# WeGoToMars/indexed_bzip2

Hardware: AMD Instinct MI355X
Metric: decompressed MB/s (whole node), 2 GiB Silesia bz2-9 (higher is better)
Workload: dtype u8

## Files before the change

indexed_bzip2_amd/csrc/bz2_hscan.hip.h:

```cpp
#pragma once

#include "bz2_stage1.hip.h"

namespace bz2gpu
{
constexpr uint32_t SCAN_LUT_BITS = 10;
constexpr uint32_t SCAN_LUT_SIZE = 1u << SCAN_LUT_BITS;
constexpr uint32_t SCAN_MAX_SPAN = 1024;
constexpr uint32_t SCAN_ROWS = SCAN_MAX_SPAN / 64;
constexpr uint32_t GROUP_SYMS = 50;
constexpr uint32_t MAX_SCAN_GROUPS = 18002;
constexpr uint32_t LEN_STOP = 0x80u;
constexpr uint32_t SYM_THREADS = 128;
constexpr uint32_t SYM_CHUNKS = 4;

struct alignas( 16 ) HuffTables
{
    uint16_t lut[6][SCAN_LUT_SIZE];
    uint16_t perm[6][264];
    uint32_t first[6][24];
    uint32_t count[6][24];
    uint32_t offs[6][24];
    uint32_t minmax[8];
};
static_assert( sizeof( HuffTables ) % 16 == 0 );

struct ScanMeta
{
    uint64_t pos_base;
    uint32_t size_bits;
    uint32_t n_groups;
    uint32_t terminal;
    uint32_t symbol_count;
    uint32_t pad[2];
};

constexpr uint32_t SCAN_RING_ENTRIES = 256;
constexpr uint32_t SCAN_RING_MIRROR = 40;

constexpr uint32_t LEV_ENTRIES = SCAN_MAX_SPAN + 16;
constexpr uint32_t LEV_BYTES = 2 * LEV_ENTRIES;

struct alignas( 16 ) ScanSlot
{
    uint16_t lev[3 * LEV_ENTRIES];

    __device__ __forceinline__ uint8_t* bytes() { return reinterpret_cast<uint8_t*>( lev ); }
    __device__ __forceinline__ uint16_t& at( uint32_t array, uint32_t entry ) { return lev[array * LEV_ENTRIES + entry]; }
};

struct ScanHeader
{
    uint64_t enc_size, pos_base;
    int32_t  status, is_eos, is_eof;
    uint32_t active, header_crc, orig_ptr, symbol_count, n_sel, size_bits, p0, n_words;
};

template<uint32_t K>
struct ScanShared
{
    uint8_t  lenlut[6][SCAN_LUT_SIZE];
    uint32_t limit[6][24];
    uint32_t eob_lo[6], eob_hi[6];
    uint32_t minmax[6];
    uint32_t ring[2 * ( SCAN_RING_ENTRIES + SCAN_RING_MIRROR )];
    ScanHeader hdr;
    union alignas( 16 ) {
        struct {
            uint16_t lut[SCAN_LUT_SIZE];
            uint32_t first[24], count[24], offs[24], running[24];
            uint16_t perm[264];
            uint16_t bitmap[16];
            uint8_t  lens[264];
            uint8_t  sym_to_byte[256];
        } build;
        ScanSlot slot[K > 1 ? 2 : 1];
    };
};

template<uint32_t RING = SCAN_RING_ENTRIES>
__device__ __forceinline__ void
ring_put( uint32_t* ring, uint32_t index, uint32_t raw )
{
    const uint32_t value = be32( raw );
    const uint32_t e1 = index & ( RING - 1 );
    const uint32_t e0 = ( index - 1 ) & ( RING - 1 );
    ring[2 * e1 + 1] = value;
    ring[2 * e0] = value;
    if ( e1 < SCAN_RING_MIRROR ) ring[2 * ( RING + e1 ) + 1] = value;
    if ( e0 < SCAN_RING_MIRROR ) ring[2 * ( RING + e0 )] = value;
}

template<uint32_t K>
__device__ __forceinline__ void
scan_sync()
{
    if ( K > 1 ) __syncthreads(); else wave_sync();
// ... 928 lines not shown
        const uint32_t fullGroups = terminal ? nGroups - 1 : nGroups;
        BlockMeta mt;
        mt.enc_off = start;
        mt.enc_size = sh.hdr.enc_size;
        mt.decoded_size = 0;
        mt.out_off = 0;
        mt.header_crc = sh.hdr.header_crc;
        mt.computed_crc = 0xFFFFFFFFu;
        mt.n = 0;
        mt.orig_ptr = sh.hdr.orig_ptr;
        mt.nsym = fullGroups * GROUP_SYMS;
        mt.is_eos = sh.hdr.is_eos;
        mt.is_eof = sh.hdr.is_eof;
        mt.status = status;
        mt.seg_stride = MIN_SEG_STRIDE;
        mt.nseg = 0;
        mt.walk_ok = 0;
        mt.cycle_len = 0;
        mt.nchain = 0;
        mt.pad = 0;
        meta[b] = mt;
        HuffMeta hm;
        hm.n_stored = fullGroups * GROUP_SYMS;
        hm.symbol_count = sh.hdr.symbol_count;
        hm.status = status;
        hm.active = active;
        hmeta[b] = hm;
        ScanMeta sm;
        sm.pos_base = posBase;
        sm.size_bits = sizeBits;
        sm.n_groups = nGroups;
        sm.terminal = terminal;
        sm.symbol_count = sh.hdr.symbol_count;
        smeta[b] = sm;
    }
}


template<uint32_t THREADS>
struct alignas( 16 ) SymShared
{
    HuffTables tabs;
    uint16_t stage[THREADS * GROUP_SYMS];
};

template<uint32_t THREADS = SYM_THREADS>
__global__ __launch_bounds__( THREADS ) void
k_hsym( const uint32_t* __restrict__   in_words,
        BlockMeta* __restrict__        meta,
        HuffMeta* __restrict__         hmeta,
        const ScanMeta* __restrict__   smeta,
        const uint8_t* __restrict__    sel_buf,
        const HuffTables* __restrict__ tab_buf,
        const uint32_t* __restrict__   gpos_buf,
        uint16_t* __restrict__         sym_buf )
{
    extern __shared__ __attribute__( ( aligned( 16 ) ) ) uint8_t ldsAtLaunch[];
    SymShared<THREADS>& sh = *reinterpret_cast<SymShared<THREADS>*>( ldsAtLaunch );
    const uint32_t b = blockIdx.y;
    const ScanMeta sm = smeta[b];
    if ( blockIdx.x * THREADS * SYM_CHUNKS >= sm.n_groups ) return;
    const uint32_t tid = threadIdx.x;
    {
        const uint4* const src = reinterpret_cast<const uint4*>( tab_buf + b );
        uint4* const dst = reinterpret_cast<uint4*>( &sh.tabs );
        for ( uint32_t k = tid; k < sizeof( HuffTables ) / 16; k += THREADS ) dst[k] = src[k];
    }
    __syncthreads();

    for ( uint32_t chunk = 0; chunk < SYM_CHUNKS; ++chunk ) {
    const uint32_t g0 = ( blockIdx.x * SYM_CHUNKS + chunk ) * THREADS;
    if ( g0 >= sm.n_groups ) return;
    const uint32_t gi = g0 + tid;
    const uint32_t eob = sm.symbol_count + 1;
    if ( gi < sm.n_groups ) {
        const uint32_t t = sel_buf[(size_t)b * SEL_STRIDE + gi];
        const uint32_t* const words = in_words + ( sm.pos_base >> 5 );
        uint32_t pos = gpos_buf[(size_t)b * GPOS_STRIDE + gi];
        const bool last = sm.terminal && gi + 1 == sm.n_groups;
        uint32_t w = pos >> 5;
        uint64_t buf = ( ( (uint64_t)be32( words[w] ) << 32 ) | be32( words[w + 1] ) ) << ( pos & 31u );
        uint32_t have = 64 - ( pos & 31u );
        w += 2;
        const uint16_t* const lut = sh.tabs.lut[t];
        const uint32_t mm = sh.tabs.minmax[t];
        const uint32_t maxLen = mm >> 8;
        uint16_t* const out = sh.stage + tid * GROUP_SYMS;
        uint32_t cnt = 0;
        int32_t status = ST_OK;
        bool finished = false;
        for ( uint32_t j = 0; j < GROUP_SYMS; ++j ) {
            if ( have <= 32 ) {
                buf |= (uint64_t)be32( words[w] ) << ( 32 - have );
                have += 32;
                ++w;
            }
            uint32_t e = lut[(uint32_t)( buf >> ( 64 - SCAN_LUT_BITS ) )];
            uint32_t len = e & 31u, sym = e >> 5;
            if ( len == 0 ) {
                const uint32_t v20 = (uint32_t)( buf >> 44 );
                for ( uint32_t l = SCAN_LUT_BITS + 1; l <= maxLen; ++l ) {
                    const uint32_t d = ( v20 >> ( 20 - l ) ) - sh.tabs.first[t][l];
                    if ( d < sh.tabs.count[t][l] ) {
                        len = l;
                        sym = sh.tabs.perm[t][sh.tabs.offs[t][l] + d];
                        break;
                    }
                }
            }
            if ( last ) {
                if ( len == 0 ) {
                    status = pos + maxLen > sm.size_bits ? ST_EOF : ST_INVALID_CODE;
                    break;
                }
                if ( pos + len > sm.size_bits ) {
                    status = ST_EOF;
                    break;
                }
            }
            pos += len;
            buf <<= len;
            have -= len;
            if ( last && sym == eob ) {
                finished = true;
                break;
            }
            out[j] = (uint16_t)sym;
            ++cnt;
        }
        if ( last ) {
            const uint32_t stored = gi * GROUP_SYMS + cnt;
            if ( !finished && status == ST_OK ) status = ST_INVALID_CODE;
            hmeta[b].n_stored = stored;
            hmeta[b].status = status;
            meta[b].nsym = stored + ( finished ? 1u : 0u );
            meta[b].status = status;
            meta[b].enc_size = sm.pos_base + pos - meta[b].enc_off;
        }
    }
    __syncthreads();
    {
        const uint32_t nHere = sm.n_groups - g0 < THREADS ? sm.n_groups - g0 : THREADS;
        const uint32_t units = ( nHere * GROUP_SYMS * 2 + 15 ) / 16;
        uint4* const dst = reinterpret_cast<uint4*>( sym_buf + (size_t)b * SYM_STRIDE + (size_t)g0 * GROUP_SYMS );
        const uint4* const src = reinterpret_cast<const uint4*>( sh.stage );
        for ( uint32_t k = tid; k < units; k += THREADS ) dst[k] = src[k];
    }
    __syncthreads();
    }
}
}
```

indexed_bzip2_amd/csrc/bz2_kernels.hip.h:

```cpp
#pragma once

#include <hip/hip_runtime.h>
#include <stdint.h>

#include "bz2_scratch.hpp"

namespace bz2gpu
{
constexpr uint32_t MAX_N = 900000;
constexpr uint32_t MIN_SEG_STRIDE = 16;
constexpr uint32_t MARK = 0x80000000u;
constexpr uint32_t LF_MASK = 0xFFFFFu;
constexpr uint32_t INVALID_OFF = 0xFFFFFFFFu;

enum Status : int32_t {
    ST_OK = 0, ST_EOF = 1, ST_BAD_MAGIC = 2, ST_RANDOMIZED = 3, ST_ORIGPTR_RANGE = 4, ST_GROUP_COUNT = 5,
    ST_SELECTOR_COUNT = 6, ST_SELECTOR_UNARY = 7, ST_CODE_LENGTH = 8, ST_HUFFMAN_LENGTHS = 9,
    ST_SELECTOR_OVERRUN = 10, ST_INVALID_CODE = 11, ST_RUN_OVERFLOW = 12, ST_DATA_OVERFLOW = 13,
    ST_ORIGPTR_DATA = 14, ST_CRC = 15
};

struct BlockMeta
{
    uint64_t enc_off;
// ... 97 lines not shown
    }

    __device__ __forceinline__ void
    skip( uint32_t k )
    {
        buf <<= k;
        n -= k;
        pos += k;
    }

    __device__ __forceinline__ uint32_t
    read( uint32_t k )
    {
        refill();
        if ( pos + k > size_bits ) {
            eof = true;
        }
        const uint32_t v = peek( k );
        skip( k );
        return v;
    }
};

__global__ __launch_bounds__( 256 ) void
k_find_magic( const uint32_t* __restrict__ words, uint64_t size_bits, uint64_t magic48,
              uint64_t* __restrict__ found, uint32_t capacity, uint32_t* __restrict__ counter )
{
    const uint64_t nStartWords = ( size_bits + 31 ) >> 5;
    const uint64_t stride = (uint64_t)gridDim.x * 256;
    for ( uint64_t w = (uint64_t)blockIdx.x * 256 + threadIdx.x; w < nStartWords; w += stride ) {
        const uint64_t hi = ( (uint64_t)be32( words[w] ) << 32 ) | be32( words[w + 1] );
        const uint64_t lo = (uint64_t)be32( words[w + 2] ) << 32;
#pragma unroll 4
        for ( uint32_t s = 0; s < 32; ++s ) {
            const uint64_t window = s == 0 ? hi : ( ( hi << s ) | ( lo >> ( 64 - s ) ) );
            if ( ( window >> 16 ) == magic48 ) {
                const uint64_t offset = w * 32 + s;
                if ( offset + 48 <= size_bits ) {
                    const uint32_t slot = atomicAdd( counter, 1u );
                    if ( slot < capacity ) found[slot] = offset;
                }
            }
        }
    }
}

__device__ __forceinline__ uint64_t
match_any( uint32_t key, int bits, bool valid )
{
    const uint64_t all = __ballot( valid );
    uint32_t lo = 0, hi = 0;
    int b = 0;
    for ( ; b + 1 < bits; b += 2 ) {
        const uint32_t minus0 = (uint32_t)__builtin_amdgcn_sbfe( (int)key, b, 1 );
        const uint32_t minus1 = (uint32_t)__builtin_amdgcn_sbfe( (int)key, b + 1, 1 );
        const uint64_t bal0 = __ballot( minus0 != 0 );
        const uint64_t bal1 = __ballot( minus1 != 0 );
        lo = lo | ( (uint32_t)bal0 ^ minus0 ) | ( (uint32_t)bal1 ^ minus1 );
        hi = hi | ( (uint32_t)( bal0 >> 32 ) ^ minus0 ) | ( (uint32_t)( bal1 >> 32 ) ^ minus1 );
    }
    if ( b < bits ) {
        const uint32_t minusBit = (uint32_t)__builtin_amdgcn_sbfe( (int)key, b, 1 );
        const uint64_t bal = __ballot( minusBit != 0 );
        lo |= (uint32_t)bal ^ minusBit;
        hi |= (uint32_t)( bal >> 32 ) ^ minusBit;
    }
    return all & ~( ( (uint64_t)hi << 32 ) | lo );
}

__device__ __forceinline__ uint64_t
match_any_runs( uint32_t key, bool valid )
{
    const uint32_t first = (uint32_t)__builtin_amdgcn_readfirstlane( (int)key );
    if ( __ballot( valid && key != first ) == 0 ) return __ballot( valid );
    return match_any( key, 8, valid );
}

__device__ __forceinline__ uint32_t
popc_below( uint64_t mask, uint32_t lane )
{
    return __popcll( mask & ( ( 1ull << lane ) - 1ull ) );
}

__global__ __launch_bounds__( 1024 ) void
k_bwt_build( const BlockMeta* __restrict__ meta,
             const uint8_t* __restrict__   l_buf,
             uint32_t* __restrict__        tab_buf )
{
    __shared__ uint32_t hist[BWT_WAVES][256];
    __shared__ uint32_t tot[256];
    const uint32_t b = blockIdx.x;
    const BlockMeta mt = meta[b];
    if ( !mt.walk_ok ) return;
    const uint32_t N = mt.n, origPtr = mt.orig_ptr, stride = mt.seg_stride;
    const uint8_t* const L = l_buf + (size_t)b * L_STRIDE;
    uint32_t* const tab = tab_buf + (size_t)b * TAB_STRIDE;
    const uint32_t tid = threadIdx.x, wave = tid >> 6, lane = tid & 63;

    uint32_t chunk = ( N + BWT_WAVES - 1 ) / BWT_WAVES;
    chunk = ( chunk + 255u ) & ~255u;
    const uint32_t begin = wave * chunk < N ? wave * chunk : N;
    const uint32_t end = begin + chunk < N ? begin + chunk : N;

    for ( uint32_t i = tid; i < BWT_WAVES * 256; i += 1024 ) ( &hist[0][0] )[i] = 0;
    __syncthreads();

    for ( uint32_t base = begin; base < end; base += 256 ) {
        const uint32_t i = base + 4 * lane;
        if ( i < end ) {
            const uint32_t v = *reinterpret_cast<const uint32_t*>( L + i );
            const uint32_t nb = end - i < 4 ? end - i : 4;
            for ( uint32_t k = 0; k < nb; ++k ) atomicAdd( &hist[wave][( v >> ( 8 * k ) ) & 0xFF], 1u );
        }
    }
    __syncthreads();
    if ( tid < 256 ) {
        uint32_t run = 0;
        for ( int w = 0; w < BWT_WAVES; ++w ) {
            const uint32_t t = hist[w][tid];
            hist[w][tid] = run;
            run += t;
        }
        tot[tid] = run;
    }
    __syncthreads();
    if ( tid < 64 ) {
        uint32_t v0 = tot[4 * tid], v1 = tot[4 * tid + 1], v2 = tot[4 * tid + 2], v3 = tot[4 * tid + 3];
        const uint32_t s = v0 + v1 + v2 + v3;
        uint32_t incl = s;
        for ( int d = 1; d < 64; d <<= 1 ) {
            const uint32_t o = __shfl_up( incl, d );
            if ( (int)tid >= d ) incl += o;
        }
        uint32_t excl = incl - s;
        tot[4 * tid] = excl; excl += v0;
        tot[4 * tid + 1] = excl; excl += v1;
        tot[4 * tid + 2] = excl; excl += v2;
        tot[4 * tid + 3] = excl;
    }
    __syncthreads();
    if ( tid < 256 ) {
        const uint32_t c = tot[tid];
        for ( int w = 0; w < BWT_WAVES; ++w ) hist[w][tid] += c;
    }
    __syncthreads();

    uint32_t rem = ( begin + lane ) % stride;
    const uint32_t remStep = 64u % stride;
    for ( uint32_t base4 = begin; base4 < end; base4 += 256 ) {
        uint32_t keys[4];
#pragma unroll
        for ( uint32_t u = 0; u < 4; ++u ) keys[u] = L[base4 + 64 * u + lane];
#pragma unroll
        for ( uint32_t u = 0; u < 4; ++u ) {
            const uint32_t i = base4 + 64 * u + lane;
            const bool valid = i < end;
            const uint32_t key = valid ? keys[u] : 0u;
            const uint64_t same = match_any_runs( key, valid );
            const uint32_t rank = popc_below( same, lane );
            uint32_t basePos = 0;
            if ( valid ) basePos = hist[wave][key];
            if ( valid ) {
                const uint32_t lf = basePos + rank;
                const bool mark = ( rem == 0 ) || ( i == origPtr );
                tab[i] = ( lf << 8 ) | key | ( mark ? MARK : 0u );
                if ( rank == 0 ) hist[wave][key] = basePos + (uint32_t)__popcll( same );
            }
            rem += remStep;
            if ( rem >= stride ) rem -= stride;
        }
    }
}

__device__ __forceinline__ void
bwt_chunk_range( uint32_t N, uint32_t slices, uint32_t slice, uint32_t wave, uint32_t& begin, uint32_t& end )
{
    uint32_t chunk = ( N + slices * BWT_WAVES - 1 ) / ( slices * BWT_WAVES );
    chunk = ( chunk + 255u ) & ~255u;
    const uint32_t index = slice * BWT_WAVES + wave;
    begin = index * chunk < N ? index * chunk : N;
    end = begin + chunk < N ? begin + chunk : N;
}

__global__ __launch_bounds__( 1024 ) void
k_bwt_count( const BlockMeta* __restrict__ meta,
             const uint8_t* __restrict__   l_buf,
             uint32_t* __restrict__        counts,
             uint32_t                      slices )
{
    __shared__ uint32_t hist[BWT_WAVES][256];
    const uint32_t b = blockIdx.y, slice = blockIdx.x;
    const BlockMeta mt = meta[b];
    if ( !mt.walk_ok ) return;
    const uint8_t* const L = l_buf + (size_t)b * L_STRIDE;
    const uint32_t tid = threadIdx.x, wave = tid >> 6, lane = tid & 63;
    uint32_t begin, end;
    bwt_chunk_range( mt.n, slices, slice, wave, begin, end );
    for ( uint32_t i = tid; i < BWT_WAVES * 256; i += 1024 ) ( &hist[0][0] )[i] = 0;
    __syncthreads();
    for ( uint32_t base = begin; base < end; base += 256 ) {
        const uint32_t i = base + 4 * lane;
        if ( i < end ) {
            const uint32_t v = *reinterpret_cast<const uint32_t*>( L + i );
            const uint32_t nb = end - i < 4 ? end - i : 4;
            for ( uint32_t k = 0; k < nb; ++k ) atomicAdd( &hist[wave][( v >> ( 8 * k ) ) & 0xFF], 1u );
        }
    }
    __syncthreads();
    uint32_t* const out = counts + (size_t)b * BWT_COUNTS_PER_BLOCK + (size_t)slice * BWT_WAVES * 256;
    for ( uint32_t i = tid; i < BWT_WAVES * 256; i += 1024 ) out[i] = ( &hist[0][0] )[i];
}

__global__ __launch_bounds__( 1024 ) void
k_bwt_rank( const BlockMeta* __restrict__ meta,
            const uint8_t* __restrict__   l_buf,
            uint32_t* __restrict__        tab_buf,
            const uint32_t* __restrict__  counts,
            uint32_t                      slices )
{
    __shared__ uint32_t hist[BWT_WAVES][256];
    __shared__ uint32_t tot[256];
    const uint32_t b = blockIdx.y, slice = blockIdx.x;
    const BlockMeta mt = meta[b];
    if ( !mt.walk_ok ) return;
    const uint32_t N = mt.n, origPtr = mt.orig_ptr, stride = mt.seg_stride;
    const uint8_t* const L = l_buf + (size_t)b * L_STRIDE;
    uint32_t* const tab = tab_buf + (size_t)b * TAB_STRIDE;
    const uint32_t tid = threadIdx.x, wave = tid >> 6, lane = tid & 63;
    if ( tid < 256 ) {
        const uint32_t* const of = counts + (size_t)b * BWT_COUNTS_PER_BLOCK + tid;
        uint32_t run = 0;
        for ( uint32_t c = 0; c < slices * BWT_WAVES; ++c ) {
            const uint32_t t = of[(size_t)c * 256];
            if ( c / BWT_WAVES == slice ) hist[c % BWT_WAVES][tid] = run;
            run += t;
        }
        tot[tid] = run;
    }
    __syncthreads();
    if ( tid < 64 ) {
        uint32_t v0 = tot[4 * tid], v1 = tot[4 * tid + 1], v2 = tot[4 * tid + 2], v3 = tot[4 * tid + 3];
        const uint32_t s4 = v0 + v1 + v2 + v3;
        uint32_t incl = s4;
        for ( int d = 1; d < 64; d <<= 1 ) {
            const uint32_t o = __shfl_up( incl, d );
            if ( (int)tid >= d ) incl += o;
        }
        uint32_t excl = incl - s4;
        tot[4 * tid] = excl; excl += v0;
        tot[4 * tid + 1] = excl; excl += v1;
        tot[4 * tid + 2] = excl; excl += v2;
        tot[4 * tid + 3] = excl;
    }
    __syncthreads();
    if ( tid < 256 ) {
        const uint32_t c = tot[tid];
        for ( int w = 0; w < BWT_WAVES; ++w ) hist[w][tid] += c;
    }
    __syncthreads();

    uint32_t begin, end;
    bwt_chunk_range( N, slices, slice, wave, begin, end );
    uint32_t rem = ( begin + lane ) % stride;
    const uint32_t remStep = 64u % stride;
    for ( uint32_t base4 = begin; base4 < end; base4 += 256 ) {
        uint32_t keys[4];
#pragma unroll
        for ( uint32_t u = 0; u < 4; ++u ) keys[u] = L[base4 + 64 * u + lane];
#pragma unroll
        for ( uint32_t u = 0; u < 4; ++u ) {
            const uint32_t i = base4 + 64 * u + lane;
            const bool valid = i < end;
            const uint32_t key = valid ? keys[u] : 0u;
            const uint64_t same = match_any_runs( key, valid );
            const uint32_t rank = popc_below( same, lane );
            uint32_t basePos = 0;
            if ( valid ) basePos = hist[wave][key];
            if ( valid ) {
                const uint32_t lf = basePos + rank;
                const bool mark = ( rem == 0 ) || ( i == origPtr );
                tab[i] = ( lf << 8 ) | key | ( mark ? MARK : 0u );
                if ( rank == 0 ) hist[wave][key] = basePos + (uint32_t)__popcll( same );
            }
            rem += remStep;
            if ( rem >= stride ) rem -= stride;
        }
    }
}

__global__ __launch_bounds__( 256 ) void
k_replicate( const BlockMeta* __restrict__ meta,
             uint8_t*                      r_buf,
             uint8_t*                      tmp_buf,
// ... 434 lines not shown
```

indexed_bzip2_amd/csrc/bz2_walk.hip.h:

```cpp
#pragma once

#include "bz2_kernels.hip.h"

namespace bz2gpu
{
constexpr uint32_t WALK_THREADS = 256;
constexpr uint32_t WALK_QUEUES = 8;
constexpr uint32_t EMIT_THREADS = 256;
constexpr uint32_t EMIT_TILES = 4;
constexpr uint32_t EMIT_STAGE = 16384;

struct WalkPlan
{
    uint32_t q_begin[WALK_QUEUES + 1];
    uint32_t q_total[WALK_QUEUES];
    uint32_t ctr[WALK_QUEUES];
    uint32_t pad[15];
};

__global__ __launch_bounds__( 256 ) void
k_walk_plan( const BlockMeta* __restrict__ meta, uint32_t n, WalkPlan* plan, uint32_t* blk, uint32_t* pre )
{
    __shared__ uint32_t begin[WALK_QUEUES + 1];
    const uint32_t t = threadIdx.x;
    if ( t == 0 ) {
        uint32_t acc = 0;
        for ( uint32_t q = 0; q < WALK_QUEUES; ++q ) {
            begin[q] = acc;
            acc += q < n ? ( n - q + WALK_QUEUES - 1 ) / WALK_QUEUES : 0;
        }
        begin[WALK_QUEUES] = acc;
    }
    __syncthreads();
    if ( t <= WALK_QUEUES ) plan->q_begin[t] = begin[t];
    if ( t < WALK_QUEUES ) {
        uint32_t idx = begin[t], acc = 0;
        for ( uint32_t i = t; i < n; i += WALK_QUEUES ) {
            blk[idx] = i;
            pre[idx] = acc;
            acc += meta[i].walk_ok ? meta[i].nseg : 0u;
            ++idx;
        }
        plan->q_total[t] = acc;
        plan->ctr[t] = 0;
    }
}

constexpr uint32_t LINK_THREADS = 256;
constexpr uint32_t LINK_SPLIT = 128;
constexpr uint32_t LINK_MAX_SUB = KMAX / LINK_SPLIT + 2;

struct alignas( 16 ) LinkShared
{
    uint16_t ssucc[SEG_STRIDE];
    uint32_t subLen[LINK_MAX_SUB];
    uint16_t subNext[LINK_MAX_SUB];
    uint32_t subOff[LINK_MAX_SUB];
    uint32_t subCnt[LINK_MAX_SUB];
    uint32_t subRank[LINK_MAX_SUB];
};

__device__ __forceinline__ void
link_block( BlockMeta*                   meta,
            const uint32_t* __restrict__ seg_len,
            const uint32_t* __restrict__ seg_succ,
            uint2* __restrict__          chain,
            uint16_t* __restrict__       ssucc,
            uint32_t* __restrict__       subLen,
            uint16_t* __restrict__       subNext,
            uint32_t* __restrict__       subOff,
            uint32_t* __restrict__       subCnt,
            uint32_t* __restrict__       subRank )
{
    const uint32_t b = blockIdx.x;
    const BlockMeta mt = meta[b];
    if ( !mt.walk_ok ) return;
    const uint32_t nseg = mt.nseg, N = mt.n, stride = mt.seg_stride, origPtr = mt.orig_ptr;
    const uint32_t k0 = ( N + stride - 1 ) / stride;
    const size_t base = (size_t)b * SEG_STRIDE;
    const uint32_t first = ( origPtr % stride != 0 ) ? k0 : origPtr / stride;
    const uint32_t tid = threadIdx.x;

    for ( uint32_t j = tid; j < nseg; j += LINK_THREADS ) {
        const uint32_t s = seg_succ[base + j];
        ssucc[j] = (uint16_t)( s < nseg ? s : 0xFFFFu );
    }
    const uint32_t nSplit = ( nseg + LINK_SPLIT - 1 ) / LINK_SPLIT;
    const bool firstExtra = first % LINK_SPLIT != 0;
    const uint32_t nSub = nSplit + ( firstExtra ? 1u : 0u );
    const auto splitterOf = [&] ( uint32_t seg ) -> uint32_t {
        if ( seg == first && firstExtra ) return nSplit;
        return seg % LINK_SPLIT == 0 ? seg / LINK_SPLIT : 0xFFFFu;
    };
    for ( uint32_t s = tid; s < LINK_MAX_SUB; s += LINK_THREADS ) subOff[s] = INVALID_OFF;
    __syncthreads();

    constexpr uint32_t AHEAD = 8;
    for ( uint32_t s = tid; s < nSub; s += LINK_THREADS ) {
        uint32_t cur = s < nSplit ? s * LINK_SPLIT : first;
        uint32_t sum = 0, steps = 0, nextSub = 0xFFFFu;
        bool more = true;
        while ( more ) {
            uint32_t nodes[AHEAD];
            uint32_t m = 0;
#pragma unroll
            for ( uint32_t k = 0; k < AHEAD; ++k ) {
                nodes[k] = cur;
                if ( more ) {
                    m = k + 1;
                    cur = ssucc[cur];
                    ++steps;
                    if ( cur == 0xFFFFu || steps > nseg ) {
                        more = false;
                    } else {
                        nextSub = splitterOf( cur );
                        more = nextSub == 0xFFFFu;
                    }
                }
            }
#pragma unroll
            for ( uint32_t k = 0; k < AHEAD; ++k ) {
                if ( k < m ) sum += seg_len[base + nodes[k]];
            }
        }
        subLen[s] = sum;
        subCnt[s] = steps;
        subNext[s] = (uint16_t)nextSub;
    }
    __syncthreads();

    if ( tid == 0 ) {
        const uint32_t start = firstExtra ? nSplit : first / LINK_SPLIT;
        uint32_t s = start, off = 0, visited = 0, rank = 0;
        bool ok = true;
        do {
            subOff[s] = off;
            subRank[s] = rank;
            off += subLen[s];
            rank += subCnt[s];
            s = subNext[s];
            ++visited;
            if ( s == 0xFFFFu || visited > nSub || off > N ) { ok = false; break; }
        } while ( s != start );
        meta[b].cycle_len = off;
        meta[b].nchain = rank;
        if ( !ok || off == 0 ) {
            meta[b].status = ST_CRC;
            meta[b].walk_ok = 0;
        }
    }
    __syncthreads();

    for ( uint32_t s = tid; s < nSub; s += LINK_THREADS ) {
        uint32_t off = subOff[s];
        if ( off == INVALID_OFF ) continue;
        uint32_t cur = s < nSplit ? s * LINK_SPLIT : first;
        uint32_t steps = 0;
        uint32_t rank = subRank[s];
        bool more = true;
        while ( more ) {
            uint32_t nodes[AHEAD], lens[AHEAD];
            uint32_t m = 0;
#pragma unroll
            for ( uint32_t k = 0; k < AHEAD; ++k ) {
                nodes[k] = cur;
                if ( more ) {
                    m = k + 1;
                    cur = ssucc[cur];
                    ++steps;
                    more = !( cur == 0xFFFFu || steps > nseg || splitterOf( cur ) != 0xFFFFu );
                }
            }
#pragma unroll
            for ( uint32_t k = 0; k < AHEAD; ++k ) lens[k] = k < m ? seg_len[base + nodes[k]] : 0u;
#pragma unroll
            for ( uint32_t k = 0; k < AHEAD; ++k ) {
                if ( k < m ) {
                    const uint32_t len = lens[k];
                    chain[base + rank] = make_uint2( off | ( nodes[k] << 20 ), len | ( ( nodes[k] >> 12 ) << 20 ) );
                    ++rank;
                    off += len;
                }
            }
        }
    }
}

__global__ __launch_bounds__( LINK_THREADS ) void
k_link2( BlockMeta*                   meta,
         const uint32_t* __restrict__ seg_len,
         const uint32_t* __restrict__ seg_succ,
         uint2* __restrict__          chain )
{
    extern __shared__ __attribute__( ( aligned( 16 ) ) ) uint8_t ldsAtLaunch[];
    auto& shared = *reinterpret_cast<LinkShared*>( ldsAtLaunch );
    link_block( meta, seg_len, seg_succ, chain, shared.ssucc, shared.subLen, shared.subNext, shared.subOff,
                shared.subCnt, shared.subRank );
}

__global__ __launch_bounds__( WALK_THREADS ) void
k_walk( const BlockMeta* __restrict__ meta,
         const uint32_t* __restrict__  tab_buf,
         WalkPlan*                     plan,
         const uint32_t* __restrict__  blk,
         const uint32_t* __restrict__  pre,
         uint32_t*                     seg_len,
         uint32_t*                     seg_succ,
         uint32_t                      chunk,
         uint32_t*                     stash,
         uint32_t*                     seg_cont )
{
    __shared__ uint32_t sBase, sNext, sK0;
    const uint32_t tid = threadIdx.x;
    const uint32_t lane = tid & 63u;
    uint32_t xcc;
    asm volatile( "s_getreg_b32 %0, hwreg(HW_REG_XCC_ID)" : "=s"( xcc ) );
    xcc &= WALK_QUEUES - 1;

    for ( uint32_t attempt = 0; attempt < WALK_QUEUES; ++attempt ) {
        const uint32_t q = ( xcc + attempt ) & ( WALK_QUEUES - 1 );
        const uint32_t qb = plan->q_begin[q], qe = plan->q_begin[q + 1];
        const uint32_t total = plan->q_total[q];
        if ( total == 0 ) continue;
        for ( ;; ) {
            __syncthreads();
            if ( tid == 0 ) {
                const uint32_t base = atomicAdd( &plan->ctr[q], chunk );
                sBase = base;
                uint32_t lo = qb, hi = qe;
                while ( hi - lo > 1 ) {
                    const uint32_t mid = ( lo + hi ) >> 1;
                    if ( pre[mid] <= base ) lo = mid; else hi = mid;
                }
                sK0 = lo;
            }
            __syncthreads();
            uint32_t base = sBase;
            if ( base >= total ) break;
            const uint32_t claimEnd = total - base < chunk ? total : base + chunk;
            uint32_t k = sK0;
            while ( base < claimEnd ) {
                while ( k + 1 < qe && base >= pre[k + 1] ) ++k;
                const uint32_t runEnd = ( k + 1 < qe && pre[k + 1] < claimEnd ) ? pre[k + 1] : claimEnd;
                const uint32_t cnt = runEnd - base;
                const uint32_t b = blk[k];
                const uint32_t j0 = base - pre[k];
                const uint32_t N = meta[b].n, stride = meta[b].seg_stride, origPtr = meta[b].orig_ptr;
                const uint32_t k0 = ( N + stride - 1 ) / stride;
                const uint32_t* const tab = tab_buf + (size_t)b * TAB_STRIDE;
                const size_t segBase = (size_t)b * SEG_STRIDE;
                uint32_t* const stashOfBlock = stash + segBase * ( STASH_BYTES / 4 );
                __syncthreads();
                if ( tid == 0 ) sNext = WALK_THREADS;
                __syncthreads();

                uint32_t my = tid;
                bool idle = true;
                uint32_t j = 0, p = 0, e = 0, len = 0, piece = 0;
                for ( ;; ) {
                    if ( idle && my < cnt ) {
                        j = j0 + my;
                        p = j < k0 ? j * stride : origPtr;
                        e = tab[p];
                        len = 0;
                        piece = 0;
                        idle = false;
                    }
                    if ( __ballot( !idle ) == 0 ) break;
                    if ( !idle ) {
                        uint32_t w[4] = { 0, 0, 0, 0 };
                        bool done = false;
                        if ( piece == STASH_BYTES / 16 ) __builtin_nontemporal_store( p, seg_cont + segBase + j );
#pragma unroll
                        for ( uint32_t i = 0; i < 16; i += 4 ) {
                            if ( !done ) {
#pragma unroll
                                for ( uint32_t s4 = i; s4 < i + 4; ++s4 ) {
                                    const uint32_t live = done ? 0u : 1u;
                                    w[s4 >> 2] |= done ? 0u : ( e & 0xFFu ) << ( 8 * ( s4 & 3u ) );
                                    len += live;
// ... 159 lines not shown
```

Before: 34560.

## Prefetch Huffman words, pack BWT histograms, and two-level parallel chain linking

Three independent changes. The Huffman symbol decoder now keeps a small register window of upcoming input words, so each refill uses a word loaded earlier instead of waiting on a fresh global load. The BWT histogram kernels replace the per-wave 256-bin atomics with 128 packed 16-bit counter pairs replicated across four copies, aiming to cut LDS atomic contention, and sum the copies when reading. The link stage uses finer splitters, has each thread walk four chains with lookahead, and adds a super-run level so the serial prefix walk on thread 0 covers far fewer nodes, falling back to the serial sub-walk when that fails; the added complexity risks correctness on edge cycles.

```diff
diff --git a/indexed_bzip2_amd/csrc/bz2_hscan.hip.h b/indexed_bzip2_amd/csrc/bz2_hscan.hip.h
--- a/indexed_bzip2_amd/csrc/bz2_hscan.hip.h
+++ b/indexed_bzip2_amd/csrc/bz2_hscan.hip.h
@@ -13,6 +13,7 @@
 constexpr uint32_t LEN_STOP = 0x80u;
 constexpr uint32_t SYM_THREADS = 128;
 constexpr uint32_t SYM_CHUNKS = 4;
+constexpr uint32_t SYM_AHEAD = 2;
 
 struct alignas( 16 ) HuffTables
 {
@@ -1107,6 +1108,9 @@
         uint64_t buf = ( ( (uint64_t)be32( words[w] ) << 32 ) | be32( words[w + 1] ) ) << ( pos & 31u );
         uint32_t have = 64 - ( pos & 31u );
         w += 2;
+        uint32_t ahead[SYM_AHEAD];
+#pragma unroll
+        for ( uint32_t k = 0; k < SYM_AHEAD; ++k ) ahead[k] = words[w + k];
         const uint16_t* const lut = sh.tabs.lut[t];
         const uint32_t mm = sh.tabs.minmax[t];
         const uint32_t maxLen = mm >> 8;
@@ -1116,8 +1120,11 @@
         bool finished = false;
         for ( uint32_t j = 0; j < GROUP_SYMS; ++j ) {
             if ( have <= 32 ) {
-                buf |= (uint64_t)be32( words[w] ) << ( 32 - have );
+                buf |= (uint64_t)be32( ahead[0] ) << ( 32 - have );
                 have += 32;
+#pragma unroll
+                for ( uint32_t k = 0; k + 1 < SYM_AHEAD; ++k ) ahead[k] = ahead[k + 1];
+                ahead[SYM_AHEAD - 1] = words[w + SYM_AHEAD];
                 ++w;
             }
             uint32_t e = lut[(uint32_t)( buf >> ( 64 - SCAN_LUT_BITS ) )];
diff --git a/indexed_bzip2_amd/csrc/bz2_kernels.hip.h b/indexed_bzip2_amd/csrc/bz2_kernels.hip.h
--- a/indexed_bzip2_amd/csrc/bz2_kernels.hip.h
+++ b/indexed_bzip2_amd/csrc/bz2_kernels.hip.h
@@ -203,13 +203,47 @@
     return __popcll( mask & ( ( 1ull << lane ) - 1ull ) );
 }
 
+constexpr uint32_t BWT_COPIES = 4;
+constexpr uint32_t BWT_COUNTER_WORDS = BWT_WAVES * BWT_COPIES * 128;
+static_assert( ( ( MAX_N + BWT_WAVES - 1 ) / BWT_WAVES + 255u ) / 256u * 256u < 65536u, "a chunk's counts fit 16 bits" );
+
+__device__ __forceinline__ void
+bwt_count_chunk( const uint8_t* __restrict__ L, uint32_t begin, uint32_t end, uint32_t* counters, uint32_t wave, uint32_t lane )
+{
+    uint32_t* const mine = counters + ( wave * BWT_COPIES + lane % BWT_COPIES ) * 128;
+    for ( uint32_t base = begin; base < end; base += 256 ) {
+        const uint32_t i = base + 4 * lane;
+        if ( i < end ) {
+            const uint32_t v = *reinterpret_cast<const uint32_t*>( L + i );
+            const uint32_t nb = end - i < 4 ? end - i : 4;
+            for ( uint32_t k = 0; k < nb; ++k ) {
+                const uint32_t c = ( v >> ( 8 * k ) ) & 0xFF;
+                atomicAdd( &mine[c & 127u], 1u << ( ( c >> 3 ) & 16u ) );
+            }
+        }
+    }
+}
+
+__device__ __forceinline__ uint32_t
+bwt_count_of( const uint32_t* counters, uint32_t wave, uint32_t c )
+{
+    uint32_t sum = 0;
+#pragma unroll
+    for ( uint32_t copy = 0; copy < BWT_COPIES; ++copy ) {
+        sum += ( counters[( wave * BWT_COPIES + copy ) * 128 + ( c & 127u )] >> ( ( c >> 3 ) & 16u ) ) & 0xFFFFu;
+    }
+    return sum;
+}
+
 __global__ __launch_bounds__( 1024 ) void
 k_bwt_build( const BlockMeta* __restrict__ meta,
              const uint8_t* __restrict__   l_buf,
              uint32_t* __restrict__        tab_buf )
 {
-    __shared__ uint32_t hist[BWT_WAVES][256];
-    __shared__ uint32_t tot[256];
+    __shared__ uint32_t lds[BWT_COUNTER_WORDS];
+    uint32_t ( * const hist )[256] = reinterpret_cast<uint32_t ( * )[256]>( lds );
+    uint32_t* const tot = lds + BWT_WAVES * 256;
+    static_assert( BWT_WAVES * 256 + 256 <= BWT_COUNTER_WORDS );
     const uint32_t b = blockIdx.x;
     const BlockMeta mt = meta[b];
     if ( !mt.walk_ok ) return;
@@ -223,26 +257,27 @@
     const uint32_t begin = wave * chunk < N ? wave * chunk : N;
     const uint32_t end = begin + chunk < N ? begin + chunk : N;
 
-    for ( uint32_t i = tid; i < BWT_WAVES * 256; i += 1024 ) ( &hist[0][0] )[i] = 0;
-    __syncthreads();
-
-    for ( uint32_t base = begin; base < end; base += 256 ) {
-        const uint32_t i = base + 4 * lane;
-        if ( i < end ) {
-            const uint32_t v = *reinterpret_cast<const uint32_t*>( L + i );
-            const uint32_t nb = end - i < 4 ? end - i : 4;
-            for ( uint32_t k = 0; k < nb; ++k ) atomicAdd( &hist[wave][( v >> ( 8 * k ) ) & 0xFF], 1u );
-        }
-    }
-    __syncthreads();
-    if ( tid < 256 ) {
-        uint32_t run = 0;
-        for ( int w = 0; w < BWT_WAVES; ++w ) {
-            const uint32_t t = hist[w][tid];
-            hist[w][tid] = run;
-            run += t;
-        }
-        tot[tid] = run;
+    for ( uint32_t i = tid; i < BWT_COUNTER_WORDS; i += 1024 ) lds[i] = 0;
+    __syncthreads();
+
+    bwt_count_chunk( L, begin, end, lds, wave, lane );
+    __syncthreads();
+    {
+        uint32_t counted[BWT_WAVES];
+        if ( tid < 256 ) {
+#pragma unroll
+            for ( uint32_t w = 0; w < BWT_WAVES; ++w ) counted[w] = bwt_count_of( lds, w, tid );
+        }
+        __syncthreads();
+        if ( tid < 256 ) {
+            uint32_t run = 0;
+#pragma unroll
+            for ( uint32_t w = 0; w < BWT_WAVES; ++w ) {
+                hist[w][tid] = run;
+                run += counted[w];
+            }
+            tot[tid] = run;
+        }
     }
     __syncthreads();
     if ( tid < 64 ) {
@@ -309,7 +344,7 @@
              uint32_t* __restrict__        counts,
              uint32_t                      slices )
 {
-    __shared__ uint32_t hist[BWT_WAVES][256];
+    __shared__ uint32_t counters[BWT_COUNTER_WORDS];
     const uint32_t b = blockIdx.y, slice = blockIdx.x;
     const BlockMeta mt = meta[b];
     if ( !mt.walk_ok ) return;
@@ -317,19 +352,12 @@
     const uint32_t tid = threadIdx.x, wave = tid >> 6, lane = tid & 63;
     uint32_t begin, end;
     bwt_chunk_range( mt.n, slices, slice, wave, begin, end );
-    for ( uint32_t i = tid; i < BWT_WAVES * 256; i += 1024 ) ( &hist[0][0] )[i] = 0;
-    __syncthreads();
-    for ( uint32_t base = begin; base < end; base += 256 ) {
-        const uint32_t i = base + 4 * lane;
-        if ( i < end ) {
-            const uint32_t v = *reinterpret_cast<const uint32_t*>( L + i );
-            const uint32_t nb = end - i < 4 ? end - i : 4;
-            for ( uint32_t k = 0; k < nb; ++k ) atomicAdd( &hist[wave][( v >> ( 8 * k ) ) & 0xFF], 1u );
-        }
-    }
+    for ( uint32_t i = tid; i < BWT_COUNTER_WORDS; i += 1024 ) counters[i] = 0;
+    __syncthreads();
+    bwt_count_chunk( L, begin, end, counters, wave, lane );
     __syncthreads();
     uint32_t* const out = counts + (size_t)b * BWT_COUNTS_PER_BLOCK + (size_t)slice * BWT_WAVES * 256;
-    for ( uint32_t i = tid; i < BWT_WAVES * 256; i += 1024 ) out[i] = ( &hist[0][0] )[i];
+    for ( uint32_t i = tid; i < BWT_WAVES * 256; i += 1024 ) out[i] = bwt_count_of( counters, i >> 8, i & 255u );
 }
 
 __global__ __launch_bounds__( 1024 ) void
diff --git a/indexed_bzip2_amd/csrc/bz2_walk.hip.h b/indexed_bzip2_amd/csrc/bz2_walk.hip.h
--- a/indexed_bzip2_amd/csrc/bz2_walk.hip.h
+++ b/indexed_bzip2_amd/csrc/bz2_walk.hip.h
@@ -47,31 +47,41 @@
 }
 
 constexpr uint32_t LINK_THREADS = 256;
-constexpr uint32_t LINK_SPLIT = 128;
+constexpr uint32_t LINK_SPLIT = 32;
+constexpr uint32_t LINK_CHAINS = 4;
+constexpr uint32_t LINK_AHEAD = 8;
 constexpr uint32_t LINK_MAX_SUB = KMAX / LINK_SPLIT + 2;
+constexpr uint32_t LINK_SUPER = 16;
+constexpr uint32_t LINK_MAX_SUPER = ( LINK_MAX_SUB + LINK_SUPER - 1 ) / LINK_SUPER + 1;
+constexpr uint32_t LINK_NONE = 0xFFFFu;
+constexpr uint32_t LINK_OFF_CYCLE = 0xFFFFFFFFu;
+static_assert( LINK_MAX_SUPER <= LINK_THREADS );
 
 struct alignas( 16 ) LinkShared
 {
     uint16_t ssucc[SEG_STRIDE];
     uint32_t subLen[LINK_MAX_SUB];
+    uint32_t subRank[LINK_MAX_SUB];
     uint16_t subNext[LINK_MAX_SUB];
-    uint32_t subOff[LINK_MAX_SUB];
-    uint32_t subCnt[LINK_MAX_SUB];
-    uint32_t subRank[LINK_MAX_SUB];
+    uint16_t subCnt[LINK_MAX_SUB];
+    uint64_t supLen[LINK_MAX_SUPER];
+    uint32_t supCnt[LINK_MAX_SUPER];
+    uint32_t supOff[LINK_MAX_SUPER];
+    uint32_t supRank[LINK_MAX_SUPER];
+    uint16_t supNext[LINK_MAX_SUPER];
+    uint32_t linked;
 };
+static_assert( sizeof( LinkShared ) <= 80 * 1024, "two workgroups share a compute unit" );
 
 __device__ __forceinline__ void
 link_block( BlockMeta*                   meta,
             const uint32_t* __restrict__ seg_len,
             const uint32_t* __restrict__ seg_succ,
             uint2* __restrict__          chain,
-            uint16_t* __restrict__       ssucc,
-            uint32_t* __restrict__       subLen,
-            uint16_t* __restrict__       subNext,
-            uint32_t* __restrict__       subOff,
-            uint32_t* __restrict__       subCnt,
-            uint32_t* __restrict__       subRank )
-{
+            LinkShared* __restrict__     shp )
+{
+    LinkShared& sh = *shp;
+    uint16_t* const ssucc = sh.ssucc;
     const uint32_t b = blockIdx.x;
     const BlockMeta mt = meta[b];
     if ( !mt.walk_ok ) return;
@@ -83,105 +93,221 @@
 
     for ( uint32_t j = tid; j < nseg; j += LINK_THREADS ) {
         const uint32_t s = seg_succ[base + j];
-        ssucc[j] = (uint16_t)( s < nseg ? s : 0xFFFFu );
+        ssucc[j] = (uint16_t)( s < nseg ? s : LINK_NONE );
     }
     const uint32_t nSplit = ( nseg + LINK_SPLIT - 1 ) / LINK_SPLIT;
     const bool firstExtra = first % LINK_SPLIT != 0;
     const uint32_t nSub = nSplit + ( firstExtra ? 1u : 0u );
     const auto splitterOf = [&] ( uint32_t seg ) -> uint32_t {
         if ( seg == first && firstExtra ) return nSplit;
-        return seg % LINK_SPLIT == 0 ? seg / LINK_SPLIT : 0xFFFFu;
+        return seg % LINK_SPLIT == 0 ? seg / LINK_SPLIT : LINK_NONE;
     };
-    for ( uint32_t s = tid; s < LINK_MAX_SUB; s += LINK_THREADS ) subOff[s] = INVALID_OFF;
-    __syncthreads();
-
-    constexpr uint32_t AHEAD = 8;
-    for ( uint32_t s = tid; s < nSub; s += LINK_THREADS ) {
-        uint32_t cur = s < nSplit ? s * LINK_SPLIT : first;
-        uint32_t sum = 0, steps = 0, nextSub = 0xFFFFu;
-        bool more = true;
-        while ( more ) {
-            uint32_t nodes[AHEAD];
-            uint32_t m = 0;
-#pragma unroll
-            for ( uint32_t k = 0; k < AHEAD; ++k ) {
-                nodes[k] = cur;
-                if ( more ) {
-                    m = k + 1;
-                    cur = ssucc[cur];
-                    ++steps;
-                    if ( cur == 0xFFFFu || steps > nseg ) {
-                        more = false;
-                    } else {
-                        nextSub = splitterOf( cur );
-                        more = nextSub == 0xFFFFu;
+    const auto startOf = [&] ( uint32_t s ) -> uint32_t { return s < nSplit ? s * LINK_SPLIT : first; };
+    const uint32_t start = firstExtra ? nSplit : first / LINK_SPLIT;
+    const uint32_t nSuper = ( nSub + LINK_SUPER - 1 ) / LINK_SUPER;
+    const bool startExtra = start % LINK_SUPER != 0;
+    const uint32_t nRuns = nSuper + ( startExtra ? 1u : 0u );
+    const auto superOf = [&] ( uint32_t s ) -> uint32_t {
+        if ( s == start && startExtra ) return nSuper;
+        return s % LINK_SUPER == 0 ? s / LINK_SUPER : LINK_NONE;
+    };
+    for ( uint32_t s = tid; s < LINK_MAX_SUB; s += LINK_THREADS ) sh.subRank[s] = LINK_OFF_CYCLE;
+    if ( tid < LINK_MAX_SUPER ) sh.supRank[tid] = LINK_OFF_CYCLE;
+    __syncthreads();
+
+    for ( uint32_t s0 = tid; s0 < nSub; s0 += LINK_THREADS * LINK_CHAINS ) {
+        uint32_t cur[LINK_CHAINS], sum[LINK_CHAINS], steps[LINK_CHAINS], nextSub[LINK_CHAINS];
+        bool more[LINK_CHAINS];
+#pragma unroll
+        for ( uint32_t c = 0; c < LINK_CHAINS; ++c ) {
+            const uint32_t s = s0 + c * LINK_THREADS;
+            more[c] = s < nSub;
+            cur[c] = startOf( s );
+            sum[c] = 0;
+            steps[c] = 0;
+            nextSub[c] = LINK_NONE;
+        }
+        bool any = true;
+        while ( any ) {
+            uint32_t nodes[LINK_CHAINS][LINK_AHEAD];
+            uint32_t m[LINK_CHAINS];
+#pragma unroll
+            for ( uint32_t c = 0; c < LINK_CHAINS; ++c ) m[c] = 0;
+#pragma unroll
+            for ( uint32_t k = 0; k < LINK_AHEAD; ++k ) {
+#pragma unroll
+                for ( uint32_t c = 0; c < LINK_CHAINS; ++c ) {
+                    nodes[c][k] = cur[c];
+                    if ( more[c] ) {
+                        m[c] = k + 1;
+                        cur[c] = ssucc[cur[c]];
+                        ++steps[c];
+                        if ( cur[c] == LINK_NONE || steps[c] > nseg ) {
+                            more[c] = false;
+                        } else {
+                            nextSub[c] = splitterOf( cur[c] );
+                            more[c] = nextSub[c] == LINK_NONE;
+                        }
                     }
                 }
             }
 #pragma unroll
-            for ( uint32_t k = 0; k < AHEAD; ++k ) {
-                if ( k < m ) sum += seg_len[base + nodes[k]];
-            }
-        }
-        subLen[s] = sum;
-        subCnt[s] = steps;
-        subNext[s] = (uint16_t)nextSub;
-    }
-    __syncthreads();
-
+            for ( uint32_t k = 0; k < LINK_AHEAD; ++k ) {
+#pragma unroll
+                for ( uint32_t c = 0; c < LINK_CHAINS; ++c ) {
+                    if ( k < m[c] ) sum[c] += seg_len[base + nodes[c][k]];
+                }
+            }
+            any = false;
+#pragma unroll
+            for ( uint32_t c = 0; c < LINK_CHAINS; ++c ) any |= more[c];
+        }
+#pragma unroll
+        for ( uint32_t c = 0; c < LINK_CHAINS; ++c ) {
+            const uint32_t s = s0 + c * LINK_THREADS;
+            if ( s < nSub ) {
+                sh.subLen[s] = sum[c];
+                sh.subCnt[s] = (uint16_t)steps[c];
+                sh.subNext[s] = (uint16_t)nextSub[c];
+            }
+        }
+    }
+    __syncthreads();
+
+    if ( tid < nRuns ) {
+        uint32_t s = tid < nSuper ? tid * LINK_SUPER : start;
+        uint64_t len = 0;
+        uint32_t cnt = 0, steps = 0, next = LINK_NONE;
+        for ( ;; ) {
+            len += sh.subLen[s];
+            cnt += sh.subCnt[s];
+            s = sh.subNext[s];
+            ++steps;
+            if ( s == LINK_NONE || steps > nSub ) break;
+            next = superOf( s );
+            if ( next != LINK_NONE ) break;
+        }
+        sh.supLen[tid] = len;
+        sh.supCnt[tid] = cnt;
+        sh.supNext[tid] = (uint16_t)next;
+    }
+    __syncthreads();
     if ( tid == 0 ) {
-        const uint32_t start = firstExtra ? nSplit : first / LINK_SPLIT;
-        uint32_t s = start, off = 0, visited = 0, rank = 0;
+        const uint32_t startRun = startExtra ? nSuper : start / LINK_SUPER;
+        uint32_t r = startRun, visited = 0;
+        uint64_t off = 0, rank = 0;
         bool ok = true;
         do {
-            subOff[s] = off;
-            subRank[s] = rank;
-            off += subLen[s];
-            rank += subCnt[s];
-            s = subNext[s];
+            sh.supOff[r] = (uint32_t)off;
+            sh.supRank[r] = (uint32_t)rank;
+            off += sh.supLen[r];
+            rank += sh.supCnt[r];
+            r = sh.supNext[r];
             ++visited;
-            if ( s == 0xFFFFu || visited > nSub || off > N ) { ok = false; break; }
-        } while ( s != start );
-        meta[b].cycle_len = off;
-        meta[b].nchain = rank;
-        if ( !ok || off == 0 ) {
-            meta[b].status = ST_CRC;
-            meta[b].walk_ok = 0;
-        }
-    }
-    __syncthreads();
-
-    for ( uint32_t s = tid; s < nSub; s += LINK_THREADS ) {
-        uint32_t off = subOff[s];
-        if ( off == INVALID_OFF ) continue;
-        uint32_t cur = s < nSplit ? s * LINK_SPLIT : first;
-        uint32_t steps = 0;
-        uint32_t rank = subRank[s];
-        bool more = true;
-        while ( more ) {
-            uint32_t nodes[AHEAD], lens[AHEAD];
-            uint32_t m = 0;
-#pragma unroll
-            for ( uint32_t k = 0; k < AHEAD; ++k ) {
-                nodes[k] = cur;
-                if ( more ) {
-                    m = k + 1;
-                    cur = ssucc[cur];
-                    ++steps;
-                    more = !( cur == 0xFFFFu || steps > nseg || splitterOf( cur ) != 0xFFFFu );
+            if ( r == LINK_NONE || visited > nRuns || off > N ) { ok = false; break; }
+        } while ( r != startRun );
+        ok = ok && off != 0;
+        sh.linked = ok ? 1u : 0u;
+        if ( ok ) {
+            meta[b].cycle_len = (uint32_t)off;
+            meta[b].nchain = (uint32_t)rank;
+        } else {
+            uint32_t s = start, off32 = 0, rank32 = 0;
+            visited = 0;
+            ok = true;
+            do {
+                off32 += sh.subLen[s];
+                rank32 += sh.subCnt[s];
+                s = sh.subNext[s];
+                ++visited;
+                if ( s == LINK_NONE || visited > nSub || off32 > N ) { ok = false; break; }
+            } while ( s != start );
+            meta[b].cycle_len = off32;
+            meta[b].nchain = rank32;
+            if ( !ok || off32 == 0 ) {
+                meta[b].status = ST_CRC;
+                meta[b].walk_ok = 0;
+            }
+            s = start;
+            off32 = rank32 = 0;
+            for ( uint32_t v = 0; v < visited && sh.subRank[s] == LINK_OFF_CYCLE; ++v ) {
+                const uint32_t len = sh.subLen[s];
+                sh.subLen[s] = off32;
+                sh.subRank[s] = rank32;
+                off32 += len;
+                rank32 += sh.subCnt[s];
+                s = sh.subNext[s];
+            }
+        }
+    }
+    __syncthreads();
+    if ( sh.linked && tid < nRuns && sh.supRank[tid] != LINK_OFF_CYCLE ) {
+        uint32_t s = tid < nSuper ? tid * LINK_SUPER : start;
+        uint32_t off = sh.supOff[tid], rank = sh.supRank[tid];
+        for ( ;; ) {
+            const uint32_t len = sh.subLen[s];
+            sh.subLen[s] = off;
+            sh.subRank[s] = rank;
+            off += len;
+            rank += sh.subCnt[s];
+            s = sh.subNext[s];
+            if ( superOf( s ) != LINK_NONE ) break;
+        }
+    }
+    __syncthreads();
+
+    for ( uint32_t s0 = tid; s0 < nSub; s0 += LINK_THREADS * LINK_CHAINS ) {
+        uint32_t cur[LINK_CHAINS], off[LINK_CHAINS], steps[LINK_CHAINS], rank[LINK_CHAINS];
+        bool more[LINK_CHAINS];
+        bool any = false;
+#pragma unroll
+        for ( uint32_t c = 0; c < LINK_CHAINS; ++c ) {
+            const uint32_t s = s0 + c * LINK_THREADS;
+            rank[c] = s < nSub ? sh.subRank[s] : LINK_OFF_CYCLE;
+            more[c] = rank[c] != LINK_OFF_CYCLE;
+            off[c] = more[c] ? sh.subLen[s] : 0u;
+            cur[c] = startOf( s );
+            steps[c] = 0;
+            any |= more[c];
+        }
+        while ( any ) {
+            uint32_t nodes[LINK_CHAINS][LINK_AHEAD], lens[LINK_CHAINS][LINK_AHEAD];
+            uint32_t m[LINK_CHAINS];
+#pragma unroll
+            for ( uint32_t c = 0; c < LINK_CHAINS; ++c ) m[c] = 0;
+#pragma unroll
+            for ( uint32_t k = 0; k < LINK_AHEAD; ++k ) {
+#pragma unroll
+                for ( uint32_t c = 0; c < LINK_CHAINS; ++c ) {
+                    nodes[c][k] = cur[c];
+                    if ( more[c] ) {
+                        m[c] = k + 1;
+                        cur[c] = ssucc[cur[c]];
+                        ++steps[c];
+                        more[c] = !( cur[c] == LINK_NONE || steps[c] > nseg || splitterOf( cur[c] ) != LINK_NONE );
+                    }
                 }
             }
 #pragma unroll
-            for ( uint32_t k = 0; k < AHEAD; ++k ) lens[k] = k < m ? seg_len[base + nodes[k]] : 0u;
-#pragma unroll
-            for ( uint32_t k = 0; k < AHEAD; ++k ) {
-                if ( k < m ) {
-                    const uint32_t len = lens[k];
-                    chain[base + rank] = make_uint2( off | ( nodes[k] << 20 ), len | ( ( nodes[k] >> 12 ) << 20 ) );
-                    ++rank;
-                    off += len;
+            for ( uint32_t k = 0; k < LINK_AHEAD; ++k ) {
+#pragma unroll
+                for ( uint32_t c = 0; c < LINK_CHAINS; ++c ) lens[c][k] = k < m[c] ? seg_len[base + nodes[c][k]] : 0u;
+            }
+#pragma unroll
+            for ( uint32_t c = 0; c < LINK_CHAINS; ++c ) {
+#pragma unroll
+                for ( uint32_t k = 0; k < LINK_AHEAD; ++k ) {
+                    if ( k < m[c] ) {
+                        const uint32_t len = lens[c][k];
+                        chain[base + rank[c]] = make_uint2( off[c] | ( nodes[c][k] << 20 ), len | ( ( nodes[c][k] >> 12 ) << 20 ) );
+                        ++rank[c];
+                        off[c] += len;
+                    }
                 }
             }
+            any = false;
+#pragma unroll
+            for ( uint32_t c = 0; c < LINK_CHAINS; ++c ) any |= more[c];
         }
     }
 }
@@ -194,8 +320,7 @@
 {
     extern __shared__ __attribute__( ( aligned( 16 ) ) ) uint8_t ldsAtLaunch[];
     auto& shared = *reinterpret_cast<LinkShared*>( ldsAtLaunch );
-    link_block( meta, seg_len, seg_succ, chain, shared.ssucc, shared.subLen, shared.subNext, shared.subOff,
-                shared.subCnt, shared.subRank );
+    link_block( meta, seg_len, seg_succ, chain, &shared );
 }
 
 __global__ __launch_bounds__( WALK_THREADS ) void
```

Result: no change. 34540 (-0.0%).
